# Dicklesworthstone/frankensearch

Hardware: AMD Instinct MI355X
Metric: queries/sec + p50 phase-1 latency, 10M×384 f16 corpus, 1/2/4/8 MI355X (higher is better)
Workload: dtype f16 x f32 -> f32 (every emitted score, in the reference's operation order); candidate filter i8 x i8 -> i32

## Files before the change

### frankensearch_amd/csrc/kernels.hpp

```cpp
#pragma once

#include <hip/hip_runtime.h>
#include <stddef.h>
#include <stdint.h>

namespace fsgpu {

typedef unsigned long long u64;

struct ScanArgs {
    const void* slab;
    const u64* live;
    const u64* allow;
    const float* queries;
    u64* partial;
    uint32_t nrows;
    uint32_t dim;
    uint32_t k;
    uint32_t row_base;
    int32_t hreduce;
    uint32_t row_stride;
};

struct MergeArgs {
// ... 135 lines not shown
    uint32_t valid_queries;
    uint32_t slab_f32;
    uint32_t rank_only;
};
constexpr uint32_t kGroupsTaken = 24;
constexpr uint32_t kGroupsTakenMax = 32;
constexpr uint32_t kGroupsRankMax = 128;
bool select_args_ok(const SelectArgs& args);
bool select_groups_args_ok(const GroupSelectArgs& args);
bool list_cut_args_ok(uint32_t nlists, uint32_t list_len);
bool two_pass_merge_args_ok(uint32_t nshards, uint32_t cc, uint32_t k);
hipError_t launch_select_groups(const GroupSelectArgs& args, int nq, hipStream_t stream);
constexpr uint32_t kSelectPool = 1024;
constexpr uint32_t kSelectMaxK = 128;
hipError_t launch_select(const SelectArgs& args, int nq, hipStream_t stream);
hipError_t launch_list_cut(const u64* lists, uint32_t nlists, uint32_t list_len, float* out, hipStream_t stream);
hipError_t launch_two_pass_merge(const u64* approx_lists, const u64* exact_lists, uint32_t nshards, uint64_t shard_pitch, uint32_t nq,
                                 uint32_t cc, uint32_t k, uint32_t out_stride, uint32_t* out_rows, float* out_scores, uint32_t* out_counts,
                                 hipStream_t stream);
hipError_t launch_prepare_queries_i8(const float* q, uint32_t nq, uint32_t nq_pad, uint32_t dim, void* qi8, float* delta,
                                     hipStream_t stream, int bits = 8);
hipError_t launch_prepare_queries_i8_filter(const float* q, uint32_t nq, uint32_t nq_pad, uint32_t dim, uint32_t q_stride,
                                            const unsigned int* slab_max_bits, const unsigned int* slab_stats, void* qi8,
                                            float* delta, hipStream_t stream, float* unit_out = nullptr, double extra_coeff = 0.0);

constexpr uint32_t kMfmaMaxSlots = 32;
constexpr uint32_t kMfmaSpillCountStride = 16;
constexpr uint32_t kWideSlots = 32;
bool scan_mfma_supported(int dim);
bool scan_wide_supported(int dim, int elem_bytes);
bool scan_wide_group_maxima_supported(int dim, int query_tiles);
int scan_wide_max_query_tiles(int dim, int elem_bytes);
hipError_t launch_scan_wide(const MfmaScanArgs& args, int query_tiles, int grid, hipStream_t stream, int* occupancy);
void note_main_pass_kernel(const char* name);
const char* last_main_pass_kernel();
int scan_mfma_waves_per_block(int shape);
int scan_mfma_rows_per_tile(int shape);
int scan_mfma_query_tiles(int shape);
int scan_mfma_max_slots(int shape);
bool scan_mfma_shape_built(int shape);
int scan_mfma_planner_shape(int requested, int elem_bytes);
hipError_t launch_scan_mfma(const MfmaScanArgs& args, int shape, int grid, hipStream_t stream, int* occupancy);
hipError_t launch_max_row_norm(const void* slab, uint32_t nrows, uint32_t dim, uint32_t row_stride_bytes, unsigned int* out_bits,
                               hipStream_t stream);
hipError_t launch_max_row_norm_f32(const float* rows, uint32_t nrows, uint32_t dim, unsigned int* out_bits, hipStream_t stream);
hipError_t launch_prepare_queries(const float* q, uint32_t nq, uint32_t nq_pad, uint32_t dim, uint32_t q_stride,
                                  const unsigned int* max_norm_bits, void* qh, float* delta, hipStream_t stream);

hipError_t launch_slab_maxabs(const void* slab_f16, size_t n_values, unsigned int* max_bits_dev, hipStream_t stream);
hipError_t launch_quantize_slab_i8(const void* slab_f16, size_t n_values, unsigned int* max_bits_dev, void* out_i8,
                                   hipStream_t stream, bool max_ready = false);
hipError_t launch_quantize_slab_4bit_levels(const void* slab_f16, size_t n_values, unsigned int* max_bits_dev, void* out_i8,
                                            hipStream_t stream, bool max_ready = false);
hipError_t launch_i8_slab_stats(const void* slab_f16, const void* slab_i8, uint32_t nrows, uint32_t dim,
                                const unsigned int* max_bits_dev, unsigned int* stats_dev, hipStream_t stream);
hipError_t launch_rotate_rows_f16(const void* rows_f16, uint32_t nrows, uint32_t dim, const double* rt, float* out, hipStream_t stream);
hipError_t launch_rotate_rows_f32(const float* rows, uint32_t nrows, uint32_t row_stride, uint32_t dim, const double* rt, float* out,
                                  hipStream_t stream);
hipError_t launch_maxabs_f32(const float* v, size_t n, unsigned int* max_bits_dev, hipStream_t stream);
hipError_t launch_quantize_f32_i8(const float* v, size_t n, const unsigned int* max_bits_dev, void* out_i8, hipStream_t stream);
hipError_t launch_i8_stats_f32(const float* rows, const void* rows_i8, uint32_t nrows, uint32_t dim, const unsigned int* max_bits_dev,
                               unsigned int* stats_dev, hipStream_t stream);
bool scan_i8_fused_supported(int dim, int kcap);
hipError_t launch_pack_slab_4bit(const void* slab_f16, uint64_t count, uint32_t dim, unsigned int* max_bits_dev,
                                 void* out_4bit, hipStream_t stream, bool max_ready = false);
bool scan_4bit_fused_supported(int dim, int kcap);
// ... 277 lines not shown
```

### frankensearch_amd/csrc/mfma_wide.hip

```cpp
#include <atomic>
#include <cstdlib>
#include <string>
#include <vector>
#include <type_traits>

#include "scan_common.hpp"

namespace fsgpu {

using namespace scan_detail;

typedef float f32x4 __attribute__((ext_vector_type(4)));
typedef int i32x4 __attribute__((ext_vector_type(4)));

namespace {

__device__ __forceinline__ void glds16(const void* gsrc, uint32_t lds_dst) {
    unsigned keep;
    asm volatile(
        "s_mov_b32 %0, m0\n\t"
        "s_mov_b32 m0, %2\n\t"
        "s_nop 0\n\t"
        "global_load_lds_dwordx4 %1, off\n\t"
        "s_mov_b32 m0, %0"
// ... 40 lines not shown
__device__ __forceinline__ int ceil_threshold(float t) {
    if (!(t <= 33554432.0f)) return 1 << 25;
    if (t < -33554432.0f) return -(1 << 25);
    return (int)ceilf(t);
}

__device__ __forceinline__ bool wave_any(bool x) { return __ballot(x) != 0; }

template <int N>
__device__ __forceinline__ void wait_vmcnt() {
    static_assert(N >= 0 && N < 64, "vmcnt is a 6-bit field");
    asm volatile("s_waitcnt vmcnt(%0)" ::"n"(N) : "memory");
}

[[maybe_unused]] __device__ __forceinline__ void flag_post(uint32_t lds_addr, int lane) {
    asm volatile("" ::: "memory");
    if (lane == 0) {
        const uint32_t one = 1;
        asm volatile("ds_add_u32 %0, %1" ::"v"(lds_addr), "v"(one) : "memory");
    }
}
[[maybe_unused]] __device__ __forceinline__ void flag_wait(uint32_t lds_addr, uint32_t target) {
    for (;;) {
        uint32_t v;
        asm volatile("ds_read_b32 %0, %1\n\ts_waitcnt lgkmcnt(0)" : "=v"(v) : "v"(lds_addr) : "memory");
        if ((uint32_t)__builtin_amdgcn_readfirstlane(v) >= target) break;
        __builtin_amdgcn_s_sleep(1);
    }
    asm volatile("" ::: "memory");
}

}

constexpr int kOptNegTau = 2, kOptSaddr = 4, kOptSplit = 8, kOptBig = 16, kOptFlags = 32;

constexpr int wide_chunk_ksteps(int KS, int QT) {
    return KS == 12 ? (QT >= 3 ? 2 : 3) : KS == 6 ? (QT >= 5 ? 1 : 3) : KS == 4 ? (QT >= 7 ? 1 : 2) : (KS >= 2 ? KS / 2 : 1);
}
constexpr bool wide_room(int ROWB, int QT) {
    const int KS = ROWB / 64;
    return QT * KS * 4 + 4 * wide_chunk_ksteps(KS, QT) * 4 + 8 * QT <= 190;
}
constexpr bool wide_split_ok(int ROWB, int EB, int QT, int OPT, int DBG) {
    const int KS = ROWB / 64;
    return (OPT & kOptSplit) != 0 && (OPT & kOptNegTau) != 0 && EB == 1 && wide_room(ROWB, QT) && ROWB < 512 && QT >= 2 && DBG != 1 &&
           QT * KS * 4 + 2 * KS * 4 + 9 * QT <= 200;
}
constexpr bool wide_big_ok(int ROWB, int EB, int QT, int NSLOT, int OPT, int DBG) {
    return (OPT & kOptBig) != 0 && wide_split_ok(ROWB, EB, QT, OPT, DBG) && (DBG == 0 || DBG == 8 || DBG >= 16) && NSLOT == 3;
}
__device__ __forceinline__ u64 sload_u64(const u64* pv) {
    const u64* p = reinterpret_cast<const u64*>((uintptr_t)uniform_u64((uint64_t)(uintptr_t)pv));
    u64 w;
#ifdef FSGPU_LAB_SLOAD_NOGLC
    asm volatile("s_load_dwordx2 %0, %1, 0x0\n\ts_waitcnt lgkmcnt(0)" : "=&s"(w) : "s"(p) : "memory");
#elif defined(FSGPU_LAB_SLOAD_SINGLE)
    asm volatile("s_load_dwordx2 %0, %1, 0x0 glc\n\ts_waitcnt lgkmcnt(0)" : "=&s"(w) : "s"(p) : "memory");
#else
    u64 w2;
    int tries = 0;
    do {
        asm volatile("s_nop 7\n\ts_load_dwordx2 %0, %2, 0x0 glc\n\ts_load_dwordx2 %1, %2, 0x0 glc\n\ts_waitcnt lgkmcnt(0)"
                     : "=&s"(w), "=&s"(w2)
                     : "s"(p)
                     : "memory");
    } while (w != w2 && ++tries < 8);
    if (w != w2) {
// ... 26 lines not shown
    r[0] = blockIdx.x;
    r[1] = (unsigned)wave;
    r[2] = wi;
    r[3] = (unsigned long long)which | ((unsigned long long)(uintptr_t)p << 8);
    r[4] = sv;
    r[5] = vv;
    r[6] = sv2;
    r[7] = vv2;
}
#endif

template <int ROWB, int EB, int QT, int NSLOT, int OPT, int DBG, int WPBT, int NQB>
__device__ __forceinline__ void scan_wide_body(MfmaScanArgs args, const int q0_wave) {
    using acc_t = std::conditional_t<EB == 2, f32x4, i32x4>;
    constexpr int WPB = WPBT, NT = WPB * 64;
    constexpr int KS = ROWB / 64;
    constexpr bool BIG = wide_big_ok(ROWB, EB, QT, NSLOT, OPT, DBG);
    constexpr bool FLAGS = BIG && (OPT & kOptFlags) != 0;
    constexpr int TR = BIG ? 128 : ROWB >= 512 ? 32 : 64;
    constexpr int RS = TR / 16;
    constexpr int NI = RS * KS;
    constexpr int PW = NI / WPB;
    static_assert(NI % WPB == 0 && PW >= 1, "a tile's DMA instructions divide evenly over the 8 waves");
    static_assert(RS % 2 == 0, "sub-tiles are consumed in pairs");
    constexpr int CK = wide_chunk_ksteps(KS, QT);
    constexpr int NCH = KS / CK;
    constexpr int NC = (RS / 2) * NCH;
    static_assert(KS % CK == 0 && NC % 2 == 0, "an even number of chunks per tile: the register double buffer starts every tile in the same phase");
    static_assert(NSLOT >= 3, "tile n is consumed while n+1 .. n+NSLOT-2 are in flight and n-1's slot is being refilled");
    constexpr bool ROOM = wide_room(ROWB, QT);
    constexpr bool NEGTAU = (OPT & kOptNegTau) != 0 && EB == 1 && ROOM;
    constexpr bool SADDR = (OPT & kOptSaddr) != 0 && ROOM;
    constexpr bool SPLIT = wide_split_ok(ROWB, EB, QT, OPT, DBG);
    constexpr bool GMAX = DBG == 7 && SPLIT && EB == 1;
    constexpr bool SK = DBG >= 16 && DBG < 32;
    constexpr bool SK_NO_DMA = DBG == 2 || (SK && (DBG & 1)), SK_NO_SYNC = SK && (DBG & 2), SK_NO_READS = SK && (DBG & 4), SK_NO_TEST = SK && (DBG & 8);
    constexpr bool AK = DBG >= 32;
    [[maybe_unused]] constexpr bool AK_NO_STORE = AK && (DBG & 1), AK_NO_ATOMIC = AK && (DBG & 2), AK_NO_BODY = AK && (DBG & 4);
    constexpr bool STAMPS = DBG == 8;
    [[maybe_unused]] unsigned long long st_loop = 0, st_bar = 0;
    static_assert(!SPLIT || (NEGTAU && RS >= 4), "the split loop runs on neg-tau accumulators over tiles of two pairs or more");
    constexpr bool NT4 = NEGTAU && !SPLIT && QT * KS * 4 + 4 * CK * 4 + 12 * QT <= 200 && QT * KS * 4 <= 96;
    constexpr int TILE_BYTES = TR * ROWB;
    constexpr int NQ = NQB;
    if (gridDim.y > 1) {
        const uint32_t grp = blockIdx.y;
        args.queries = static_cast<const unsigned char*>(args.queries) + (size_t)grp * NQ * ROWB;
        args.tau += (size_t)grp * NQ;
        args.cand += (size_t)grp * NQ * gridDim.x * args.slots;
        if (args.cand_count) args.cand_count += (size_t)grp * NQ * gridDim.x;
        args.spill += (size_t)grp * NQ * args.spill_cap;
        args.spill_count += (size_t)grp * NQ * kMfmaSpillCountStride;
        args.overflow += (size_t)grp * NQ;
        if (!args.side_by_side) args.reverse ^= grp & 1u;
    }
    extern __shared__ __attribute__((aligned(1024))) unsigned char smem[];
    const uint32_t ring = (uint32_t)(uintptr_t)smem;
    int* lcnt = reinterpret_cast<int*>(smem + (size_t)NSLOT * TILE_BYTES);
    const uint32_t flags = ring + (uint32_t)(NSLOT * TILE_BYTES + NQ * 4);
    const int tid = threadIdx.x, lane = tid & 63;
    const int wave = __builtin_amdgcn_readfirstlane(tid >> 6);
    const int frow = lane & 15, fk = lane >> 4;
    const int slots = (int)args.slots;
    for (int i = tid; i < NQ; i += NT) lcnt[i] = 0;
    if (FLAGS && tid < 8) lcnt[NQ + tid] = 0;
    if (STAMPS && tid < 32) lcnt[NQ + 16 + tid] = 0;
// ... 136 lines not shown
#pragma unroll
        for (int h = 0; h < 2; ++h)
#pragma unroll
            for (int r = 0; r < 4; ++r) {
                if constexpr (EB == 2) m = __builtin_fmaxf(m, acc[h][nt][r]);
                else m = acc[h][nt][r] > m ? acc[h][nt][r] : m;
            }
        return m;
    };
    auto passes = [&](int nt, auto v) {
        if constexpr (NEGTAU) return v >= 0;
        else return (float)v >= tau[nt];
    };
    auto score_of = [&](int nt, auto v) {
        if constexpr (NEGTAU) return (float)(v + ctau[nt]);
        else return (float)v;
    };
    auto any_passes = [&](const acc_t (&acc)[2][QT], int nt_lo, int nt_hi) {
        bool any = false;
        if constexpr (NEGTAU) {
            int m = lane_max(acc, nt_lo);
#pragma unroll
            for (int nt = nt_lo + 1; nt < nt_hi; ++nt) {
                const int x = lane_max(acc, nt);
                m = x > m ? x : m;
            }
            any = m >= 0;
        } else {
#pragma unroll
            for (int nt = nt_lo; nt < nt_hi; ++nt) any |= passes(nt, lane_max(acc, nt));
        }
        return any;
    };
    auto emit_tiles = [&](uint32_t t, int sp, const acc_t (&acc)[2][QT], int nt_lo, int nt_hi) {
#ifdef FSGPU_EXPERIMENTS
        if constexpr (DBG == 2 || DBG == 4 || DBG == 5 || SK) {
            lcnt[q0 + frow] = 0;
            return;
        }
#endif
        if (t >= ntiles) return;
        [[maybe_unused]] unsigned long long st_in = 0;
        if constexpr (STAMPS) st_in = __builtin_readcyclecounter();
#ifdef FSGPU_LAB_APPEND_PRIO
        __builtin_amdgcn_s_setprio(FSGPU_LAB_APPEND_PRIO);
#endif
        const uint32_t pair_row0 = __builtin_amdgcn_readfirstlane(tile_row0(t) + sp * 16);
        uint32_t ok32 = pair_row0 + 32u <= args.nrows ? ~0u : pair_row0 >= args.nrows ? 0u : (1u << (args.nrows - pair_row0)) - 1u;
        if (args.live || args.allow) {
            uint32_t wi = pair_row0 >> 6;
            wi = __builtin_amdgcn_readfirstlane(wi < (last_row >> 6) ? wi : (last_row >> 6));
            u64 mask = ~0ull;
#ifdef FSGPU_LAB_VECTOR_BITMAP
            if (args.live) mask &= __builtin_nontemporal_load(args.live + wi);
            if (args.allow) mask &= __builtin_nontemporal_load(args.allow + wi);
#elif defined(FSGPU_LAB_BITMAP_CHECK)
            if (args.live) {
                const u64 sv = sload_u64(args.live + wi);
                bm_check(args.live + wi, sv, wi, 0, wave);
                mask &= sv;
            }
            if (args.allow) {
                const u64 sv = sload_u64(args.allow + wi);
                bm_check(args.allow + wi, sv, wi, 1, wave);
                mask &= sv;
            }
#else
            if (args.live) mask &= sload_u64(args.live + wi);
            if (args.allow) mask &= sload_u64(args.allow + wi);
#endif
            ok32 &= (uint32_t)(mask >> (pair_row0 & 32u));
        }
        uint32_t fk_v = (uint32_t)fk, frow_v = (uint32_t)frow, list_v = list0;
        asm volatile("" : "+v"(fk_v), "+v"(frow_v), "+v"(list_v));
        const uint32_t below_mask = (1u << fk_v) - 1u;
        const uint32_t row00 = pair_row0 + fk_v * 4u;
        unsigned char* const cand_bytes = reinterpret_cast<unsigned char*>(args.cand);
        auto take = [&](int nt, int h, int r, bool pass, u64 vote) __attribute__((always_inline)) {
            const uint32_t vlo = (uint32_t)vote >> frow_v, vhi = (uint32_t)(vote >> 32) >> frow_v;
// ... 12 lines not shown
                }
            }
            const uint32_t now = have + (uint32_t)__builtin_popcount(col);
            lcount = (lcount & ~(63u << (6 * nt))) | ((now < 63u ? now : 63u) << (6 * nt));
        };
        if (__builtin_expect(ok32 == ~0u, 1)) {
#pragma unroll
            for (int nt = nt_lo; nt < nt_hi; ++nt) {
                if (!wave_any(passes(nt, lane_max(acc, nt)))) continue;
#pragma unroll
                for (int h = 0; h < 2; ++h)
#pragma unroll
                    for (int r = 0; r < 4; ++r) {
                        const bool pass = passes(nt, acc[h][nt][r]);
                        const u64 vote = __ballot(pass);
                        if (__builtin_expect(vote != 0, 0)) take(nt, h, r, pass, vote);
                    }
            }
        } else {
            const uint32_t lb = ok32 >> (fk_v * 4u);
#pragma unroll
            for (int nt = nt_lo; nt < nt_hi; ++nt) {
                if (!wave_any(passes(nt, lane_max(acc, nt)))) continue;
#pragma unroll
                for (int h = 0; h < 2; ++h)
#pragma unroll
                    for (int r = 0; r < 4; ++r) {
                        const bool pass = passes(nt, acc[h][nt][r]) && ((lb >> (h * 16 + r)) & 1u);
                        const u64 vote = __ballot(pass);
                        if (__builtin_expect(vote != 0, 0)) take(nt, h, r, pass, vote);
                    }
            }
        }
#ifdef FSGPU_LAB_APPEND_PRIO
        __builtin_amdgcn_s_setprio(0);
#endif
        if constexpr (STAMPS) {
            const unsigned long long dt = __builtin_readcyclecounter() - st_in;
            if (lane == 0) {
                unsigned long long* st = reinterpret_cast<unsigned long long*>(lcnt + NQ + 16) + wave * 2;
                atomicAdd(st, dt);
                atomicAdd(st + 1, 1ull);
            }
        }
    };
    auto emit_pair = [&](uint32_t t, int sp, const acc_t (&acc)[2][QT]) {
        if (__builtin_expect(wave_any(any_passes(acc, 0, QT)), 0)) emit_tiles(t, sp, acc, 0, QT);
    };

#ifndef FSGPU_LAB_NO_DCACHE_INV
    if (args.live || args.allow) asm volatile("s_dcache_inv\n\ts_waitcnt lgkmcnt(0)" ::: "memory");
#endif
    __syncthreads();
    Cursor cl{0, blockIdx.x, blockIdx.x};
    Cursor cc = cl;
    auto fetch_part = [&](uint32_t slot, int part) {
        uint32_t t = cl.n < rounds ? cursor_tile(cl) : ntiles;
        t = t < ntiles ? t : ntiles - 1;
        issue_part(t, slot, part);
        if (part == PARTS - 1 && cl.n < rounds) cursor_next(cl);
    };
    auto fetch_next = [&](uint32_t slot) {
#pragma unroll
        for (int part = 0; part < PARTS; ++part) fetch_part(slot, part);
    };
#pragma unroll
    for (int j = 0; j < NSLOT - 1; ++j) fetch_next((uint32_t)j);
    if constexpr (SPLIT) {
        constexpr int NP = RS / 2;
        constexpr int QA = QT / 2;
        half8 f[2][KS];
        acc_t acc[2][QT];
        [[maybe_unused]] bool sk_loop = false;
        auto read_frag = [&](const unsigned char* base, int pair, int kk) {
            if constexpr (SK_NO_READS) {
                if (sk_loop) {
#pragma unroll
                    for (int h = 0; h < 2; ++h) asm volatile("" : "+v"(f[h][kk]));
                    return;
                }
// ... 68 lines not shown
                        for (int nt = nt_lo; nt < nt_hi; ++nt) {
                            int v = -0x7fffffff - 1;
#pragma unroll
                            for (int h = 0; h < 2; ++h)
#pragma unroll
                                for (int rr = 0; rr < 4; ++rr) {
                                    const int x = keep[h][rr] ? acc[h][nt][rr] : -0x7fffffff - 1;
                                    v = x > v ? x : v;
                                }
                            const bool better = v > gbest[nt];
                            gbest[nt] = better ? v : gbest[nt];
                            grow[nt] = better ? g : grow[nt];
                        }
                    } else {
#pragma unroll
                        for (int nt = nt_lo; nt < nt_hi; ++nt) {
                            const int v = lane_max(acc, nt);
                            const bool better = v > gbest[nt];
                            gbest[nt] = better ? v : gbest[nt];
                            grow[nt] = better ? g : grow[nt];
                        }
                    }
                }
            }
        };
        if constexpr (STAMPS) st_loop = __builtin_readcyclecounter();
        while (cc.n < rounds) {
            const uint32_t slot_next = slot + 1 == NSLOT ? 0 : slot + 1;
            const unsigned char* nxt = slot_base(slot_next);
            const uint32_t t = cursor_tile(cc);
#pragma unroll
            for (int p = 0; p < NP; ++p) {
                constexpr int TK = KS >= 4 ? 2 : 0;
                init_acc(0, QA);
                bool anyB = false;
#pragma unroll
                for (int kk = 0; kk < KS; ++kk) {
                    mfma_step(kk, 0, QA);
                    if constexpr (GMAX) {
                        if (kk == TK) gmax_update(tB, ((p + NP - 1) % NP) * 2, QA, QT);
                    } else {
                        if (kk == TK) anyB = sk_any(QA, QT);
                    }
                    if (p == 0 && kk == 0 && !SK_NO_SYNC) {
                        [[maybe_unused]] unsigned long long st_a = 0;
                        if constexpr (STAMPS) st_a = __builtin_readcyclecounter();
                        wait_vmcnt<PW*(NSLOT - 3)>();
                        if constexpr (FLAGS) {
                            flag_post(flags + slot_next * 4, lane);
                        } else {
                            __builtin_amdgcn_s_barrier();
                            asm volatile("" ::: "memory");
                        }
                        if constexpr (STAMPS) st_bar += __builtin_readcyclecounter() - st_a;
                    }
                    {
                        constexpr int IPP = (PARTS + NP - 1) / NP;
                        constexpr int K1 = KS >= 3 ? 2 : KS - 1, K2 = KS >= 5 ? 4 : K1;
                        if constexpr (FLAGS) {
                            if (p == 0 && kk == K1 && cc.n >= 1) flag_wait(flags + 16 + slot_prev * 4, WPB * ((cc.n - 1) / NSLOT + 1));
                        }
                        if (kk == K1 && p * IPP < PARTS) fetch_part(slot_prev, p * IPP);
                        if (IPP > 1 && K2 != K1 && kk == K2 && p * IPP + 1 < PARTS) fetch_part(slot_prev, p * IPP + 1);
                    }
                    __builtin_amdgcn_sched_barrier(0);
                }
                if (__builtin_expect(wave_any(anyB), 0)) emit_tiles(tB, ((p + NP - 1) % NP) * 2, acc, QA, QT);
                init_acc(QA, QT);
                bool anyA = false;
#pragma unroll
                for (int kk = 0; kk < KS; ++kk) {
                    mfma_step(kk, QA, QT);
                    if constexpr (FLAGS) {
                        if (p + 1 == NP && kk == 0) flag_wait(flags + slot_next * 4, WPB * ((cc.n + 1) / NSLOT + 1));
                    }
                    if (p + 1 < NP) read_frag(cur, p + 1, kk);
                    else read_frag(nxt, 0, kk);
                    if constexpr (GMAX) {
                        if (kk == TK) gmax_update(t, p * 2, 0, QA);
                    } else {
                        if (kk == TK) anyA = sk_any(0, QA);
                    }
                    __builtin_amdgcn_sched_barrier(0);
                }
                if constexpr (FLAGS) {
                    if (p + 2 == NP) flag_post(flags + 16 + slot * 4, lane);
                }
                if (__builtin_expect(wave_any(anyA), 0)) emit_tiles(t, p * 2, acc, 0, QA);
                tB = t;
            }
            cursor_next(cc);
            slot_prev = slot;
            slot = slot_next;
            cur = nxt;
        }
        if constexpr (GMAX) {
            gmax_update(tB, (NP - 1) * 2, QA, QT);
            wait_vmcnt<0>();
#pragma unroll
            for (int nt = 0; nt < QT; ++nt) {
                const u64 e = gbest[nt] == -0x7fffffff - 1 ? kEmpty : pack((float)gbest[nt], args.row_base + grow[nt] + (uint32_t)fk * 4u);
                args.cand[((size_t)(q0 + nt * 16 + frow) * gridDim.x + blockIdx.x) * 4 + fk] = e;
            }
            __syncthreads();
            return;
        } else {
            if (__builtin_expect(wave_any(any_passes(acc, QA, QT)), 0)) emit_tiles(tB, (NP - 1) * 2, acc, QA, QT);
        }
    } else {
    half8 fa[2][2][CK];
    wait_vmcnt<PW*(NSLOT - 2)>();
    __builtin_amdgcn_s_barrier();
    asm volatile("" ::: "memory");
    read_chunk(slot_base(0), 0, fa[0]);
#ifdef FSGPU_EXPERIMENTS
    if constexpr (DBG == 5) {
        read_chunk(slot_base(0), 1, fa[1]);
        frag_ready = true;
    }
#endif
    uint32_t slot = 0, slot_prev = NSLOT - 1;
    const unsigned char* cur = slot_base(0);
    while (cc.n < rounds) {
        const uint32_t slot_next = slot + 1 == NSLOT ? 0 : slot + 1;
        const unsigned char* nxt = slot_base(slot_next);
        const uint32_t t = cursor_tile(cc);
        acc_t acc[2][QT];
#pragma unroll
        for (int c = 0; c < NC; ++c) {
            if (c % NCH == 0) {
#pragma unroll
                for (int h = 0; h < 2; ++h)
#pragma unroll
                    for (int nt = 0; nt < QT; ++nt) {
                        if constexpr (NT4) acc[h][nt] = ntau4[nt];
                        else if constexpr (NEGTAU) acc[h][nt] = acc_t{-ctau[nt], -ctau[nt], -ctau[nt], -ctau[nt]};
                        else acc[h][nt] = acc_t{0, 0, 0, 0};
                    }
            }
            if (c + 1 < NC) read_chunk(cur, c + 1, fa[(c + 1) & 1]);
// ... 47 lines not shown
        if (j >= lcnt[q]) args.cand[((size_t)q * gridDim.x + blockIdx.x) * slots + j] = kEmpty;
    }
}

template <int ROWB, int EB, int QT, int NSLOT, int OPT, int DBG = 0>
__global__ __launch_bounds__(512) void scan_wide_kernel(MfmaScanArgs args) {
    scan_wide_body<ROWB, EB, QT, NSLOT, OPT, DBG, 8, 8 * QT * 16>(args, __builtin_amdgcn_readfirstlane((int)(threadIdx.x >> 6)) * QT * 16);
}

template <int ROWB, int EB, int QTA, int QTB, int NSLOT, int OPT>
__global__ __launch_bounds__(512) void scan_wide_asym_kernel(MfmaScanArgs args) {
    const int wave = __builtin_amdgcn_readfirstlane((int)(threadIdx.x >> 6));
    if (wave < 4) scan_wide_body<ROWB, EB, QTA, NSLOT, OPT, 0, 8, 64 * (QTA + QTB)>(args, wave * QTA * 16);
    else scan_wide_body<ROWB, EB, QTB, NSLOT, OPT, 0, 8, 64 * (QTA + QTB)>(args, 64 * QTA + (wave - 4) * QTB * 16);
}


namespace {

#ifdef FSGPU_WIDE_OPT_DEFAULT
constexpr int kWideOptDefault = FSGPU_WIDE_OPT_DEFAULT;
#else
constexpr int kWideOptDefault = kOptNegTau | kOptSaddr | kOptSplit | kOptBig;
#endif

#ifdef FSGPU_EXPERIMENTS
int wide_env(const char* name) {
    const char* e = std::getenv(name);
    return e ? std::atoi(e) : -1;
}
#endif

template <int ROWB, int EB, int QT, int NSLOT, int OPT, int DBG = 0>
hipError_t launch_wide_t(const MfmaScanArgs& args, int grid, hipStream_t stream, int* occupancy) {
    constexpr bool BIG = wide_big_ok(ROWB, EB, QT, NSLOT, OPT, DBG);
    constexpr int TR = BIG ? 128 : ROWB >= 512 ? 32 : 64;
    constexpr size_t ring = (size_t)NSLOT * TR * ROWB;
    const size_t lds = ring + (size_t)QT * 128 * 4 + 64 + (DBG == 8 ? 256 : 0);
    auto kern = scan_wide_kernel<ROWB, EB, QT, NSLOT, OPT, DBG>;
    static bool attr_done = false;
    if (!attr_done) {
        hipError_t e = hipFuncSetAttribute(reinterpret_cast<const void*>(kern), hipFuncAttributeMaxDynamicSharedMemorySize, (int)lds);
        if (e != hipSuccess) return e;
        attr_done = true;
    }
    if (occupancy) {
        int blocks = 0;
        if (hipOccupancyMaxActiveBlocksPerMultiprocessor(&blocks, kern, 512, lds) != hipSuccess || blocks < 1) blocks = 1;
        *occupancy = blocks;
        return hipSuccess;
    }
    if (args.slots > kWideSlots) return hipErrorInvalidValue;
    static const std::string name = "scan_wide_kernel<" + std::to_string(ROWB) + ", " + std::to_string(EB) + ", " +
                                    std::to_string(QT) + ", " + std::to_string(NSLOT) + ", " + std::to_string(OPT) + ">";
    if (DBG != 3 && DBG != 7) note_main_pass_kernel(name.c_str());
    hipLaunchKernelGGL(kern, dim3(grid, args.groups ? args.groups : 1), dim3(512), lds, stream, args);
    return hipGetLastError();
}

#ifdef FSGPU_LAB_ASYM
template <int ROWB, int EB, int QTA, int QTB, int NSLOT, int OPT>
hipError_t launch_wide_asym(const MfmaScanArgs& args, int grid, hipStream_t stream) {
    constexpr size_t ring = (size_t)NSLOT * 64 * ROWB;
    const size_t lds = ring + (size_t)64 * (QTA + QTB) * 4 + 64;
    auto kern = scan_wide_asym_kernel<ROWB, EB, QTA, QTB, NSLOT, OPT>;
    static bool attr_done = false;
    if (!attr_done) {
        hipError_t e = hipFuncSetAttribute(reinterpret_cast<const void*>(kern), hipFuncAttributeMaxDynamicSharedMemorySize, (int)lds);
        if (e != hipSuccess) return e;
        attr_done = true;
    }
    if (args.slots > kWideSlots) return hipErrorInvalidValue;
    note_main_pass_kernel("scan_wide_kernel<384, 1, asym>");
    hipLaunchKernelGGL(kern, dim3(grid, args.groups ? args.groups : 1), dim3(512), lds, stream, args);
    return hipGetLastError();
}
#endif

template <int ROWB, int EB, int QT, int NSLOT, int O, int MODE>
hipError_t launch_wide_pick(const MfmaScanArgs& args, int grid, hipStream_t stream, int* occupancy) {
    if constexpr (MODE == 0 && wide_big_ok(ROWB, EB, QT, 3, O, 0)) return launch_wide_t<ROWB, EB, QT, 3, O, 0>(args, grid, stream, occupancy);
    else return launch_wide_t<ROWB, EB, QT, NSLOT, O & ~(kOptBig | kOptFlags), MODE>(args, grid, stream, occupancy);
}

template <int EB, int QT, int MODE = 0>
hipError_t launch_wide_d(const MfmaScanArgs& args, int grid, hipStream_t stream, int* occupancy) {
    if (QT * (int)(args.dim * EB / 64) * 4 > 144) return hipErrorInvalidValue;
    constexpr int O = kWideOptDefault;
    switch (args.dim * EB / 2) {
        case 384: if constexpr (QT <= 3 && MODE != 7) {
#ifdef FSGPU_EXPERIMENTS
            if constexpr (MODE == 0 && EB == 2 && QT == 2) {
                static const int dbg = wide_env("FSGPU_WIDE_DBG");
                if (dbg == 1) return launch_wide_t<768, EB, QT, 6, O, 1>(args, grid, stream, occupancy);
                if (dbg == 2) return launch_wide_t<768, EB, QT, 6, O, 2>(args, grid, stream, occupancy);
            }
#endif
            return launch_wide_t<768, EB, QT, 6, O & ~(kOptBig | kOptFlags), MODE>(args, grid, stream, occupancy);
        } else return hipErrorInvalidValue;
        case 256: if constexpr (QT <= 4 && MODE != 7) return launch_wide_t<512, EB, QT, 8, O & ~kOptFlags, MODE>(args, grid, stream, occupancy);
                  else return hipErrorInvalidValue;
        case 192: if constexpr (EB != 1 || (MODE == 7 && !wide_split_ok(384, 1, QT, O, 7))) return hipErrorInvalidValue; else {
#ifdef FSGPU_EXPERIMENTS
            if constexpr (EB == 1 && QT == 4) {
                static const int opt = wide_env("FSGPU_WIDE_OPT");
                static const int dbg = wide_env("FSGPU_WIDE_DBG");
                if constexpr (MODE == 0) {
                    if (dbg == 1) return launch_wide_t<384, EB, QT, 6, 6, 1>(args, grid, stream, occupancy);
                    if (dbg == 2) return launch_wide_t<384, EB, QT, 6, 6, 2>(args, grid, stream, occupancy);
                    if (dbg == 4) return launch_wide_t<384, EB, QT, 6, 6, 4>(args, grid, stream, occupancy);
                    if (dbg == 5) return launch_wide_t<384, EB, QT, 6, 6, 5>(args, grid, stream, occupancy);
                }
                switch (opt) {
                    case 0: return launch_wide_t<384, EB, QT, 6, 0, MODE>(args, grid, stream, occupancy);
                    case 2: return launch_wide_t<384, EB, QT, 6, 2, MODE>(args, grid, stream, occupancy);
                    case 4: return launch_wide_t<384, EB, QT, 6, 4, MODE>(args, grid, stream, occupancy);
                    case 6: return launch_wide_t<384, EB, QT, 6, 6, MODE>(args, grid, stream, occupancy);
                    case 14: return launch_wide_t<384, EB, QT, 6, 14, MODE>(args, grid, stream, occupancy);
                    case 30:
                        if constexpr (MODE == 0) return launch_wide_t<384, EB, QT, 3, 30, MODE>(args, grid, stream, occupancy);
                        else return launch_wide_t<384, EB, QT, 6, 14, MODE>(args, grid, stream, occupancy);
// ... 25 lines not shown
                            slow[half] += S;
                            ent[half] += E;
                            int b = (int)(10.0 * B / L);
                            ++hist[b < 0 ? 0 : b > 9 ? 9 : b];
                        }
                        std::fprintf(stderr, "[wide stamps] waves %zu  loop cycles/wave %.0f | at the tile's wait + barrier: waves 0-3 %.1f %%, waves 4-7 %.1f %% | in the append path: "
                                             "%.1f %% / %.1f %% (%.0f / %.0f entries per wave, %.0f cycles each) | waves by barrier share, deciles:",
                                     nwaves, loop / nwaves, 100 * bar[0] / lp[0], 100 * bar[1] / lp[1], 100 * slow[0] / lp[0], 100 * slow[1] / lp[1],
                                     ent[0] / (nwaves / 2), ent[1] / (nwaves / 2), (slow[0] + slow[1]) / std::max(1.0, ent[0] + ent[1]));
                        for (int b = 0; b < 10; ++b) std::fprintf(stderr, " %d", hist[b]);
                        std::fprintf(stderr, "\n");
                        return hipSuccess;
                    }
                    switch (dbg) {
#define FSGPU_SK(D) case D: return launch_wide_t<384, EB, QT, 3, O, D>(args, grid, stream, occupancy);
                        FSGPU_SK(16) FSGPU_SK(17) FSGPU_SK(18) FSGPU_SK(20) FSGPU_SK(24) FSGPU_SK(31) FSGPU_SK(33) FSGPU_SK(35) FSGPU_SK(36)
#undef FSGPU_SK
                        default: break;
                    }
                }
            }
#endif
#ifdef FSGPU_LAB_ASYM
            if constexpr (EB == 1 && QT == 4 && MODE == 0) { if (!occupancy) return launch_wide_asym<384, 1, FSGPU_LAB_ASYM, 8 - FSGPU_LAB_ASYM, 6, O & ~(kOptBig | kOptFlags)>(args, grid, stream); }
#endif
            return launch_wide_pick<384, EB, QT, 6, O, MODE>(args, grid, stream, occupancy);
        }
        case 128: if constexpr (EB != 1 || (MODE == 7 && !wide_split_ok(256, 1, QT, O, 7))) return hipErrorInvalidValue;
                  else return launch_wide_pick<256, EB, QT, 8, O, MODE>(args, grid, stream, occupancy);
        default: return hipErrorInvalidValue;
    }
}

}

#ifdef FSGPU_LAB_BITMAP_CHECK
extern "C" int fsgpu_lab_bitmap_debug(unsigned long long* out, int cap_records) {
    unsigned int n = 0;
    if (hipMemcpyFromSymbol(&n, HIP_SYMBOL(g_bm_dbg_n), 4) != hipSuccess) return -1;
    const int take = (int)(n < 64u ? n : 64u) < cap_records ? (int)(n < 64u ? n : 64u) : cap_records;
    if (take > 0 && hipMemcpyFromSymbol(out, HIP_SYMBOL(g_bm_dbg), (size_t)take * 64) != hipSuccess) return -1;
    return (int)n;
}
#endif

bool scan_wide_supported(int dim, int elem_bytes) {
    const int rowb = dim * elem_bytes;
    return rowb == 768 || rowb == 512 || (elem_bytes == 1 && (rowb == 384 || rowb == 256));
}

bool scan_wide_group_maxima_supported(int dim, int query_tiles) {
    return (dim == 384 || dim == 256) && query_tiles >= 2 && query_tiles <= 5 &&
           wide_split_ok(dim, 1, query_tiles, kWideOptDefault, 7);
}

int scan_wide_max_query_tiles(int dim, int elem_bytes) {
    const int per_tile = dim * elem_bytes / 64 * 4;
    const int fit = per_tile > 0 ? 144 / per_tile : 0;
    if (elem_bytes != 1) return fit > 3 ? 3 : fit;
    return fit > 5 ? 5 : fit;
}

hipError_t launch_scan_wide(const MfmaScanArgs& args, int query_tiles, int grid, hipStream_t stream, int* occupancy) {
    const int eb = args.elem_bytes == 1 ? 1 : 2;
    if (!scan_wide_supported((int)args.dim, eb) || query_tiles > scan_wide_max_query_tiles((int)args.dim, eb)) return hipErrorInvalidValue;
    const bool sample = args.group_count != 0;
// ... 22 lines not shown
```

### frankensearch_amd/csrc/vector_index_batched.cpp

```cpp
#include "vector_index.hpp"

#include <algorithm>
#include <cmath>
#include <cstdio>
#include <cstdlib>
#include <chrono>
#include <cstring>

#include "../../include/fsgpu.h"
#include "lab_env.hpp"
#include "vector_index_internal.hpp"

namespace fsgpu {

using namespace detail;

SearchError VectorIndex::search_top_k_batched_device(const float* queries_dev, uint32_t nq, uint32_t query_len,
                                                     uint32_t k, const uint64_t* allow_dev, uint32_t* out_rows_dev,
                                                     float* out_scores_dev, uint32_t* out_counts_dev,
                                                     hipStream_t stream, uint32_t* fallbacks, uint64_t* out_packed_dev) {
    BatchedRequest rq(queries_dev, nq, query_len, k, stream);
    rq.allow_dev = allow_dev;
    rq.out_rows_dev = out_rows_dev;
    rq.out_scores_dev = out_scores_dev;
    rq.out_counts_dev = out_counts_dev;
    rq.out_packed_dev = out_packed_dev;
    BatchedOutcome o;
    const SearchError e = batched_exact(rq, &o);
    if (fallbacks) *fallbacks = o.fallbacks;
    return e;
}

SearchError VectorIndex::batched_exact(BatchedRequest& rq, BatchedOutcome* out) {
    const uint32_t nq = rq.nq, k = rq.k;
    const bool strided = !dense_rows();
    bool i8f = batched_filter != 1 && (batched_filter == 2 || !i8f_disabled_) && !strided && variant == 0 && knobs().filter != 1 &&
               scan_mfma_supported((int)dim_) && k >= 1 && k <= 64 && nrows_ >= 4 * 8192ull;
    if (batched_filter == 0 && knobs().filter == 0 && nq < 16 && !filter_ready() && !int8_latency) i8f = false;
    if (i8f && !filter_ready()) {
        FSGPU_TRY(ensure_filter_copy(rq.stream));
        if (!filter_ready()) i8f = false;
    }
    rq.i8_filter = i8f;
    FSGPU_TRY(batched_impl(rq, out));
    if (i8f && out->parked) tickets_[rq.ticket].i8f = true;
    else if (i8f) i8f_account(nq, f32_ ? out->fallbacks : out->refiltered);
    return ok();
}
// ... 565 lines not shown
    a = MfmaScanArgs{};
    a.slab = p.i8f ? filter_slab() : i8 ? (p.rq.bits == 4 ? n4u_slab_.ptr : i8_slab_.ptr) : slab_dev_;
    a.elem_bytes = i8 ? 1 : 2;
    a.live = reinterpret_cast<const u64*>(live_dev_);
    a.allow = reinterpret_cast<const u64*>(p.rq.allow_dev);
    a.queries = mf_qh_.ptr;
    a.tau = p.tau;
    a.cand = r.cand;
    a.spill = p.spill;
    a.spill_count = p.spill_count;
    a.spill_cap = BatchedPlan::SPILL;
    a.overflow = r.overflow;
    a.dim = dim_;
    a.row_stride = p.strided ? row_stride_ : 0;
    a.row_base = (uint32_t)row_base_;
    a.nrows = p.N;
    r.short_stages = nrows_ < 4'000'000;
    r.anchor = p.i8f && !knobs().no_anchor;
    return ok();
}

SearchError VectorIndex::batched_sample(const BatchedPlan& p, BatchedRound& r) {
    constexpr uint32_t SPILL = BatchedPlan::SPILL;
    hipStream_t stream = p.rq.stream;
    const bool i8 = p.i8, i8f = p.i8f, skip_b = p.skip_b;
    const uint32_t N = p.N, RA = p.RA, RB = p.RB, QP = r.QP, ksel = p.ksel;
    MfmaScanArgs& a = r.a;
    const uint32_t groups_a = RA / 64, groups_b = RB / 64;
    const uint32_t stride_b = (N / 64) / groups_b;
    const bool rank_groups = i8 && !i8f && ksel <= kGroupsRankMax;
    const bool group_sample = (r.anchor ? ksel <= kGroupsTakenMax : rank_groups) && r.wide_qt != 0 && !skip_b && !knobs().no_wide_b &&
                              !knobs().no_group_sample && (dim_ & 7) == 0 && dim_ <= 1024 && scan_wide_group_maxima_supported((int)dim_, r.wide_qt);
    if (group_sample) {
        const int grid_g = std::min(r.wide_grid, (int)std::max<uint32_t>(1, RB / 64 / 4));
        const uint32_t entries = (uint32_t)grid_g * 4;
        const bool extended = r.anchor ? ksel > kGroupsTaken : ksel > 64;
        if (grid_g * 4 <= 1024 && entries >= (r.anchor ? 96u : 4u * std::min(ksel, 64u)) && (!extended || entries >= 1024)) {
            MfmaScanArgs c = a;
            c.dense = nullptr;
            c.stage = 3;
            c.group_stride = stride_b;
            c.group_count = groups_b;
            c.slots = 4;
            c.groups = r.ngroups / r.wide_mult;
            c.queries = mf_qh_.ptr;
            c.tau = p.tau;
            c.cand = r.cand;
            c.cand_count = nullptr;
            c.spill = p.spill;
            c.spill_count = p.spill_count;
            c.overflow = r.overflow;
            FSGPU_HIP(launch_scan_wide(c, r.wide_qt, grid_g, stream, nullptr));
            GroupSelectArgs g{};
            g.groups = r.cand;
            g.nentries = (uint32_t)grid_g * 4;
            g.k = ksel;
            g.delta = p.delta;
            g.anchor_unit = p.unit;
            g.tau_out = p.tau;
            g.overflow = r.overflow;
            g.spill_reset = p.spill_count;
            g.slab = slab_dev_;
            g.live = a.live;
            g.allow = a.allow;
            g.queries = r.qg;
            g.dim = dim_;
            g.nrows = N;
            g.row_base = (uint32_t)row_base_;
            g.query_stride = p.qs;
            g.hreduce = hreduce;
            g.slab_f32 = f32_ ? 1u : 0u;
            g.valid_queries = r.ng;
            g.rank_only = r.anchor ? 0u : 1u;
            FSGPU_HIP(launch_select_groups(g, (int)QP, stream));
            a.dense = nullptr;
            a.stage = 1;
            a.group_stride = stride_b;
// ... 490 lines not shown
```

### frankensearch_amd/csrc/vector_index_internal.hpp

```cpp
#pragma once

#include <algorithm>
#include <cstdint>
#include <cstdlib>
#include <cstring>
#include <string>
#include <utility>

#include "../../include/fsgpu.h"
#include "vector_index.hpp"

namespace fsgpu {
namespace detail {

inline SearchError ok() { return SearchError{}; }

inline SearchError hip_fail(hipError_t e, const char* what) {
    SearchError err;
    err.code = FSGPU_ERR_DEVICE;
    err.detail = std::string(what) + ": " + hipGetErrorString(e);
    return err;
}

inline SearchError make_error(int32_t code, std::string detail) {
// ... 2 lines not shown
    e.detail = std::move(detail);
    return e;
}

inline uint32_t crc32_ieee(const uint8_t* p, size_t n) {
    static uint32_t table[256];
    static bool init = false;
    if (!init) {
        for (uint32_t i = 0; i < 256; ++i) {
            uint32_t c = i;
            for (int b = 0; b < 8; ++b) c = (c & 1u) ? (0xedb88320u ^ (c >> 1)) : (c >> 1);
            table[i] = c;
        }
        init = true;
    }
    uint32_t c = 0xffffffffu;
    for (size_t i = 0; i < n; ++i) c = table[(c ^ p[i]) & 0xffu] ^ (c >> 8);
    return ~c;
}

inline uint64_t fnv1a(const char* p, size_t n) {
    uint64_t h = 0xcbf29ce484222325ull;
    for (size_t i = 0; i < n; ++i) {
        h ^= (uint8_t)p[i];
        h *= 0x100000001b3ull;
    }
    return h;
}

struct Knobs {
    int grid_blocks = 0, ra = 0, rb = 0, mfma_shape = 0, mfma_shape_i8 = 0, round = 0, i8_per_cu = 0;
    int wide = -1;
    bool wide_sequential = false;
    int filter = 0;
    int slots_b = 0, slots_main = 0;
    int wide_max = 0;
    int i8f_growth = 0;
    bool no_skip_b = false, use_160 = false, debug_batched = false, no_reverse = false, no_wide_b = false, no_anchor = false;
    bool no_big_pool = false, no_heur_b = false, no_group_sample = false;
    bool narrow_i8f = false;
    int rb_pct = 0;
    int heur_rank = 0;
    int wide_min = 0;
    Knobs() {
        auto env = [](const char* name) { return std::getenv(name); };
        if (const char* w = env("FSGPU_WIDE")) wide = std::atoi(w);
        if (const char* l = env("FSGPU_WIDE_LAYOUT")) wide_sequential = std::strcmp(l, "sequential") == 0;
        if (const char* f = env("FSGPU_FILTER")) filter = std::strcmp(f, "f16") == 0 ? 1 : std::strcmp(f, "i8") == 0 ? 2 : 0;
        debug_batched = env("FSGPU_DEBUG_BATCHED") != nullptr;
#ifdef FSGPU_EXPERIMENTS
        auto num = [&](const char* name) {
            const char* e = env(name);
            return e ? std::atoi(e) : 0;
        };
        grid_blocks = num("FSGPU_GRID_BLOCKS");
        ra = num("FSGPU_RA");
        rb = num("FSGPU_RB");
        rb_pct = num("FSGPU_RB_PCT");
        round = num("FSGPU_ROUND");
        i8_per_cu = num("FSGPU_I8_PER_CU");
        mfma_shape = num("FSGPU_MFMA_SHAPE");
        mfma_shape_i8 = num("FSGPU_MFMA_SHAPE_I8");
        i8f_growth = num("FSGPU_I8F_GROWTH");
        wide_max = num("FSGPU_WIDE_MAX");
        wide_min = num("FSGPU_WIDE_MIN");
        slots_b = std::min(num("FSGPU_SLOTS_B"), (int)kWideSlots);
        slots_main = std::min(num("FSGPU_SLOTS_MAIN"), (int)kWideSlots);
        no_skip_b = env("FSGPU_NO_SKIP_B") != nullptr;
        no_wide_b = env("FSGPU_NO_WIDE_B") != nullptr;
        no_anchor = env("FSGPU_NO_ANCHOR") != nullptr;
        no_big_pool = env("FSGPU_NO_BIG_POOL") != nullptr;
        no_heur_b = env("FSGPU_NO_HEUR_B") != nullptr;
        no_group_sample = env("FSGPU_NO_GROUP_SAMPLE") != nullptr;
        narrow_i8f = env("FSGPU_NARROW_I8F") != nullptr;
        heur_rank = num("FSGPU_HEUR_RANK");
        no_reverse = env("FSGPU_NO_REVERSE") != nullptr;
        use_160 = env("FSGPU_USE_160") != nullptr;
#endif
    }
};
// ... 104 lines not shown
```

Baseline: 364,800.

## Stagger wave priorities in split wide scan and run group sampling side by side

Inside the split wide scan loop, each wave now raises or lowers its hardware priority (s_setprio) according to its position in the tile pass, and goes to top priority while emitting candidates. The aim is to stagger waves so MFMA work and DMA or emit phases overlap instead of colliding. Separately, the group-maxima sampling stage can now use a side-by-side layout, with fewer walkers per group when the grid divides evenly. An env knob turns the priority staggering off, and side_by_side depends on a new args field whose handling in the kernel is not shown.

```diff
diff --git a/frankensearch_amd/csrc/kernels.hpp b/frankensearch_amd/csrc/kernels.hpp
--- a/frankensearch_amd/csrc/kernels.hpp
+++ b/frankensearch_amd/csrc/kernels.hpp
@@ -191,6 +191,7 @@
 bool scan_wide_group_maxima_supported(int dim, int query_tiles);
 int scan_wide_max_query_tiles(int dim, int elem_bytes);
 hipError_t launch_scan_wide(const MfmaScanArgs& args, int query_tiles, int grid, hipStream_t stream, int* occupancy);
+bool scan_wide_flat_priority();
 void note_main_pass_kernel(const char* name);
 const char* last_main_pass_kernel();
 int scan_mfma_waves_per_block(int shape);
diff --git a/frankensearch_amd/csrc/mfma_wide.hip b/frankensearch_amd/csrc/mfma_wide.hip
--- a/frankensearch_amd/csrc/mfma_wide.hip
+++ b/frankensearch_amd/csrc/mfma_wide.hip
@@ -96,7 +96,9 @@
 
 }
 
-constexpr int kOptNegTau = 2, kOptSaddr = 4, kOptSplit = 8, kOptBig = 16, kOptFlags = 32;
+constexpr int kOptNegTau = 2, kOptSaddr = 4, kOptSplit = 8, kOptBig = 16, kOptFlags = 32, kOptFlat = 64;
+
+constexpr int wide_level(int h, int H) { return 3 - (h * 4) / H; }
 
 constexpr int wide_chunk_ksteps(int KS, int QT) {
     return KS == 12 ? (QT >= 3 ? 2 : 3) : KS == 6 ? (QT >= 5 ? 1 : 3) : KS == 4 ? (QT >= 7 ? 1 : 2) : (KS >= 2 ? KS / 2 : 1);
@@ -189,6 +191,7 @@
     constexpr bool NEGTAU = (OPT & kOptNegTau) != 0 && EB == 1 && ROOM;
     constexpr bool SADDR = (OPT & kOptSaddr) != 0 && ROOM;
     constexpr bool SPLIT = wide_split_ok(ROWB, EB, QT, OPT, DBG);
+    constexpr bool LEVEL = SPLIT && (OPT & kOptFlat) == 0;
     constexpr bool GMAX = DBG == 7 && SPLIT && EB == 1;
     constexpr bool SK = DBG >= 16 && DBG < 32;
     constexpr bool SK_NO_DMA = DBG == 2 || (SK && (DBG & 1)), SK_NO_SYNC = SK && (DBG & 2), SK_NO_READS = SK && (DBG & 4), SK_NO_TEST = SK && (DBG & 8);
@@ -391,7 +394,17 @@
         }
         return any;
     };
-    auto emit_tiles = [&](uint32_t t, int sp, const acc_t (&acc)[2][QT], int nt_lo, int nt_hi) {
+    auto set_level = [&](int level) __attribute__((always_inline)) {
+        if constexpr (LEVEL) {
+            switch (level) {
+                case 0: __builtin_amdgcn_s_setprio(0); break;
+                case 1: __builtin_amdgcn_s_setprio(1); break;
+                case 2: __builtin_amdgcn_s_setprio(2); break;
+                default: __builtin_amdgcn_s_setprio(3); break;
+            }
+        }
+    };
+    auto emit_tiles = [&](uint32_t t, int sp, const acc_t (&acc)[2][QT], int nt_lo, int nt_hi, int back) {
 #ifdef FSGPU_EXPERIMENTS
         if constexpr (DBG == 2 || DBG == 4 || DBG == 5 || SK) {
             lcnt[q0 + frow] = 0;
@@ -401,9 +414,13 @@
         if (t >= ntiles) return;
         [[maybe_unused]] unsigned long long st_in = 0;
         if constexpr (STAMPS) st_in = __builtin_readcyclecounter();
+        if constexpr (LEVEL) {
+            set_level(3);
+        } else {
 #ifdef FSGPU_LAB_APPEND_PRIO
-        __builtin_amdgcn_s_setprio(FSGPU_LAB_APPEND_PRIO);
-#endif
+            __builtin_amdgcn_s_setprio(FSGPU_LAB_APPEND_PRIO);
+#endif
+        }
         const uint32_t pair_row0 = __builtin_amdgcn_readfirstlane(tile_row0(t) + sp * 16);
         uint32_t ok32 = pair_row0 + 32u <= args.nrows ? ~0u : pair_row0 >= args.nrows ? 0u : (1u << (args.nrows - pair_row0)) - 1u;
         if (args.live || args.allow) {
@@ -482,9 +499,13 @@
                     }
             }
         }
+        if constexpr (LEVEL) {
+            set_level(back);
+        } else {
 #ifdef FSGPU_LAB_APPEND_PRIO
-        __builtin_amdgcn_s_setprio(0);
-#endif
+            __builtin_amdgcn_s_setprio(0);
+#endif
+        }
         if constexpr (STAMPS) {
             const unsigned long long dt = __builtin_readcyclecounter() - st_in;
             if (lane == 0) {
@@ -495,7 +516,7 @@
         }
     };
     auto emit_pair = [&](uint32_t t, int sp, const acc_t (&acc)[2][QT]) {
-        if (__builtin_expect(wave_any(any_passes(acc, 0, QT)), 0)) emit_tiles(t, sp, acc, 0, QT);
+        if (__builtin_expect(wave_any(any_passes(acc, 0, QT)), 0)) emit_tiles(t, sp, acc, 0, QT, 0);
     };
 
 #ifndef FSGPU_LAB_NO_DCACHE_INV
@@ -630,6 +651,9 @@
 #pragma unroll
             for (int p = 0; p < NP; ++p) {
                 constexpr int TK = KS >= 4 ? 2 : 0;
+                constexpr int H = 2 * NP;
+                const int lv1 = wide_level(2 * p, H), lv2 = wide_level(2 * p + 1, H);
+                if (lv1 != wide_level((2 * p + H - 1) % H, H)) set_level(lv1);
                 init_acc(0, QA);
                 bool anyB = false;
 #pragma unroll
@@ -663,7 +687,8 @@
                     }
                     __builtin_amdgcn_sched_barrier(0);
                 }
-                if (__builtin_expect(wave_any(anyB), 0)) emit_tiles(tB, ((p + NP - 1) % NP) * 2, acc, QA, QT);
+                if (__builtin_expect(wave_any(anyB), 0)) emit_tiles(tB, ((p + NP - 1) % NP) * 2, acc, QA, QT, lv1);
+                if (lv2 != lv1) set_level(lv2);
                 init_acc(QA, QT);
                 bool anyA = false;
 #pragma unroll
@@ -684,7 +709,7 @@
                 if constexpr (FLAGS) {
                     if (p + 2 == NP) flag_post(flags + 16 + slot * 4, lane);
                 }
-                if (__builtin_expect(wave_any(anyA), 0)) emit_tiles(t, p * 2, acc, 0, QA);
+                if (__builtin_expect(wave_any(anyA), 0)) emit_tiles(t, p * 2, acc, 0, QA, lv2);
                 tB = t;
             }
             cursor_next(cc);
@@ -703,7 +728,7 @@
             __syncthreads();
             return;
         } else {
-            if (__builtin_expect(wave_any(any_passes(acc, QA, QT)), 0)) emit_tiles(tB, (NP - 1) * 2, acc, QA, QT);
+            if (__builtin_expect(wave_any(any_passes(acc, QA, QT)), 0)) emit_tiles(tB, (NP - 1) * 2, acc, QA, QT, 0);
         }
     } else {
     half8 fa[2][2][CK];
@@ -817,7 +842,7 @@
 #endif
 
 template <int ROWB, int EB, int QT, int NSLOT, int OPT, int DBG = 0>
-hipError_t launch_wide_t(const MfmaScanArgs& args, int grid, hipStream_t stream, int* occupancy) {
+hipError_t launch_wide_k(const MfmaScanArgs& args, int grid, hipStream_t stream, int* occupancy) {
     constexpr bool BIG = wide_big_ok(ROWB, EB, QT, NSLOT, OPT, DBG);
     constexpr int TR = BIG ? 128 : ROWB >= 512 ? 32 : 64;
     constexpr size_t ring = (size_t)NSLOT * TR * ROWB;
@@ -841,6 +866,11 @@
     if (DBG != 3 && DBG != 7) note_main_pass_kernel(name.c_str());
     hipLaunchKernelGGL(kern, dim3(grid, args.groups ? args.groups : 1), dim3(512), lds, stream, args);
     return hipGetLastError();
+}
+
+template <int ROWB, int EB, int QT, int NSLOT, int OPT, int DBG = 0>
+hipError_t launch_wide_t(const MfmaScanArgs& args, int grid, hipStream_t stream, int* occupancy) {
+    return launch_wide_k<ROWB, EB, QT, NSLOT, wide_split_ok(ROWB, EB, QT, OPT, DBG) ? OPT : (OPT & ~kOptFlat), DBG>(args, grid, stream, occupancy);
 }
 
 #ifdef FSGPU_LAB_ASYM
@@ -868,10 +898,9 @@
     else return launch_wide_t<ROWB, EB, QT, NSLOT, O & ~(kOptBig | kOptFlags), MODE>(args, grid, stream, occupancy);
 }
 
-template <int EB, int QT, int MODE = 0>
-hipError_t launch_wide_d(const MfmaScanArgs& args, int grid, hipStream_t stream, int* occupancy) {
+template <int EB, int QT, int MODE, int O>
+hipError_t launch_wide_o(const MfmaScanArgs& args, int grid, hipStream_t stream, int* occupancy) {
     if (QT * (int)(args.dim * EB / 64) * 4 > 144) return hipErrorInvalidValue;
-    constexpr int O = kWideOptDefault;
     switch (args.dim * EB / 2) {
         case 384: if constexpr (QT <= 3 && MODE != 7) {
 #ifdef FSGPU_EXPERIMENTS
@@ -963,6 +992,12 @@
     }
 }
 
+template <int EB, int QT, int MODE = 0>
+hipError_t launch_wide_d(const MfmaScanArgs& args, int grid, hipStream_t stream, int* occupancy) {
+    if (scan_wide_flat_priority()) return launch_wide_o<EB, QT, MODE, kWideOptDefault | kOptFlat>(args, grid, stream, occupancy);
+    return launch_wide_o<EB, QT, MODE, kWideOptDefault>(args, grid, stream, occupancy);
+}
+
 }
 
 #ifdef FSGPU_LAB_BITMAP_CHECK
diff --git a/frankensearch_amd/csrc/vector_index_batched.cpp b/frankensearch_amd/csrc/vector_index_batched.cpp
--- a/frankensearch_amd/csrc/vector_index_batched.cpp
+++ b/frankensearch_amd/csrc/vector_index_batched.cpp
@@ -14,6 +14,8 @@
 namespace fsgpu {
 
 using namespace detail;
+
+bool scan_wide_flat_priority() { return knobs().wide_flat_priority; }
 
 SearchError VectorIndex::search_top_k_batched_device(const float* queries_dev, uint32_t nq, uint32_t query_len,
                                                      uint32_t k, const uint64_t* allow_dev, uint32_t* out_rows_dev,
@@ -645,17 +647,24 @@
     const bool group_sample = (r.anchor ? ksel <= kGroupsTakenMax : rank_groups) && r.wide_qt != 0 && !skip_b && !knobs().no_wide_b &&
                               !knobs().no_group_sample && (dim_ & 7) == 0 && dim_ <= 1024 && scan_wide_group_maxima_supported((int)dim_, r.wide_qt);
     if (group_sample) {
-        const int grid_g = std::min(r.wide_grid, (int)std::max<uint32_t>(1, RB / 64 / 4));
+        int grid_g = std::min(r.wide_grid, (int)std::max<uint32_t>(1, RB / 64 / 4));
+        const bool extended = r.anchor ? ksel > kGroupsTaken : ksel > 64;
+        const uint32_t entries_min = r.anchor ? 96u : 4u * std::min(ksel, 64u);
+        const uint32_t sample_groups = r.ngroups / r.wide_mult;
+        const uint32_t walkers = sample_groups > 1 && (uint32_t)grid_g % sample_groups == 0 ? (uint32_t)grid_g / sample_groups : 0;
+        const bool side_by_side = walkers != 0 && walkers % 8 == 0 && groups_b >= walkers * 4 && !knobs().wide_sequential && !extended &&
+                                  grid_g * 4 <= 1024 && walkers * 4 >= entries_min;
+        if (side_by_side) grid_g = (int)walkers;
         const uint32_t entries = (uint32_t)grid_g * 4;
-        const bool extended = r.anchor ? ksel > kGroupsTaken : ksel > 64;
-        if (grid_g * 4 <= 1024 && entries >= (r.anchor ? 96u : 4u * std::min(ksel, 64u)) && (!extended || entries >= 1024)) {
+        if (grid_g * 4 <= 1024 && entries >= entries_min && (!extended || entries >= 1024)) {
             MfmaScanArgs c = a;
             c.dense = nullptr;
             c.stage = 3;
             c.group_stride = stride_b;
             c.group_count = groups_b;
             c.slots = 4;
-            c.groups = r.ngroups / r.wide_mult;
+            c.groups = sample_groups;
+            c.side_by_side = side_by_side;
             c.queries = mf_qh_.ptr;
             c.tau = p.tau;
             c.cand = r.cand;
diff --git a/frankensearch_amd/csrc/vector_index_internal.hpp b/frankensearch_amd/csrc/vector_index_internal.hpp
--- a/frankensearch_amd/csrc/vector_index_internal.hpp
+++ b/frankensearch_amd/csrc/vector_index_internal.hpp
@@ -58,6 +58,7 @@
     int grid_blocks = 0, ra = 0, rb = 0, mfma_shape = 0, mfma_shape_i8 = 0, round = 0, i8_per_cu = 0;
     int wide = -1;
     bool wide_sequential = false;
+    bool wide_flat_priority = false;
     int filter = 0;
     int slots_b = 0, slots_main = 0;
     int wide_max = 0;
@@ -72,6 +73,7 @@
         auto env = [](const char* name) { return std::getenv(name); };
         if (const char* w = env("FSGPU_WIDE")) wide = std::atoi(w);
         if (const char* l = env("FSGPU_WIDE_LAYOUT")) wide_sequential = std::strcmp(l, "sequential") == 0;
+        if (const char* o = env("FSGPU_WIDE_PRIO")) wide_flat_priority = std::strcmp(o, "off") == 0;
         if (const char* f = env("FSGPU_FILTER")) filter = std::strcmp(f, "f16") == 0 ? 1 : std::strcmp(f, "i8") == 0 ? 2 : 0;
         debug_batched = env("FSGPU_DEBUG_BATCHED") != nullptr;
 #ifdef FSGPU_EXPERIMENTS
```

New measurement: 376,200, median of 6. 1.03x the previous value.
